# dusk-network/schnorr

Hardware: NVIDIA B200
Metric: verifies_per_s (higher is better)
Workload: dtype u32

## Files before the change

schnorr_b200/csrc/fq.cuh:

```cuda
#pragma once
#include <cstdint>

#include "constants_gen.cuh"

#if defined(__CUDACC__)
#define SB_HD __host__ __device__ __forceinline__
#define SB_D __device__ __forceinline__
#else
#define SB_HD inline
#define SB_D inline
#endif

namespace sb200 {

#ifndef SB_Q1_SHORTCUT
#define SB_Q1_SHORTCUT 0
#endif

struct fq {
  uint32_t v[8];
};

#if !defined(__CUDA_ARCH__)
namespace emu {
struct counters { unsigned long long wide, fq_mul, fq_sqr, fq_addsub, fr_mul, fq_dot5, dfma, fd_mul, fd_sqr, fd_dot5; };
inline counters& cnt() { static thread_local counters c = {}; return c; }
#define SB_COUNT(field, k) (::sb200::emu::cnt().field += (k))
static inline uint32_t add_at(uint32_t* acc, int n, int at, uint64_t val, uint32_t cin) {
  unsigned __int128 carry = cin;
  for (int i = at; i < n; i++) {
    unsigned __int128 t = (unsigned __int128)acc[i] + carry;
    if (i == at) t += (uint32_t)val;
    if (i == at + 1) t += (uint32_t)(val >> 32);
    acc[i] = (uint32_t)t;
    carry = t >> 32;
  }
  return (uint32_t)carry;
}
}
#else
#define SB_COUNT(field, k) ((void)0)
#endif

SB_HD void blk_fold_mac_odd(uint32_t& x0, uint32_t xf, uint32_t tprev, uint32_t* y, uint32_t a, uint32_t b1, uint32_t b3,
                            uint32_t b5, uint32_t b7) {
#if defined(__CUDA_ARCH__)
  asm("{\n\t.reg .u32 t;\n\t"
      "add.cc.u32 t, %10, 0xffffffff;\n\t"
      "addc.cc.u32 %0, %0, %9;\n\t"
      "madc.lo.cc.u32 %1, %11, %12, %1;\n\t"
      "madc.hi.cc.u32 %2, %11, %12, %2;\n\t"
      "madc.lo.cc.u32 %3, %11, %13, %3;\n\t"
      "madc.hi.cc.u32 %4, %11, %13, %4;\n\t"
      "madc.lo.cc.u32 %5, %11, %14, %5;\n\t"
      "madc.hi.cc.u32 %6, %11, %14, %6;\n\t"
      "madc.lo.cc.u32 %7, %11, %15, %7;\n\t"
      "madc.hi.u32 %8, %11, %15, %8;\n\t}"
      : "+r"(x0), "+r"(y[0]), "+r"(y[1]), "+r"(y[2]), "+r"(y[3]), "+r"(y[4]), "+r"(y[5]), "+r"(y[6]), "+r"(y[7])
      : "r"(xf), "r"(tprev), "r"(a), "r"(b1), "r"(b3), "r"(b5), "r"(b7));
#else
  SB_COUNT(wide, 4);
  uint64_t t = (uint64_t)x0 + xf + (tprev != 0 ? 1u : 0u);
  x0 = (uint32_t)t;
  uint32_t c = (uint32_t)(t >> 32);
  c = emu::add_at(y, 8, 0, (uint64_t)a * b1, c);
  c += emu::add_at(y, 8, 2, (uint64_t)a * b3, 0);
  c += emu::add_at(y, 8, 4, (uint64_t)a * b5, 0);
  c += emu::add_at(y, 8, 6, (uint64_t)a * b7, 0);
  (void)c;
#endif
}

SB_HD void blk_mac_even(uint32_t* x, uint32_t& ytop, uint32_t a, uint32_t b0, uint32_t b2, uint32_t b4, uint32_t b6) {
#if defined(__CUDA_ARCH__)
  asm("mad.lo.cc.u32 %0, %9, %10, %0;\n\t"
      "madc.hi.cc.u32 %1, %9, %10, %1;\n\t"
      "madc.lo.cc.u32 %2, %9, %11, %2;\n\t"
      "madc.hi.cc.u32 %3, %9, %11, %3;\n\t"
      "madc.lo.cc.u32 %4, %9, %12, %4;\n\t"
      "madc.hi.cc.u32 %5, %9, %12, %5;\n\t"
      "madc.lo.cc.u32 %6, %9, %13, %6;\n\t"
      "madc.hi.cc.u32 %7, %9, %13, %7;\n\t"
      "addc.u32 %8, %8, 0;"
      : "+r"(x[0]), "+r"(x[1]), "+r"(x[2]), "+r"(x[3]), "+r"(x[4]), "+r"(x[5]), "+r"(x[6]), "+r"(x[7]), "+r"(ytop)
      : "r"(a), "r"(b0), "r"(b2), "r"(b4), "r"(b6));
#else
  SB_COUNT(wide, 4);
  uint32_t c = emu::add_at(x, 8, 0, (uint64_t)a * b0, 0);
  c += emu::add_at(x, 8, 2, (uint64_t)a * b2, 0);
  c += emu::add_at(x, 8, 4, (uint64_t)a * b4, 0);
  c += emu::add_at(x, 8, 6, (uint64_t)a * b6, 0);
  ytop += c;
#endif
}

SB_HD void blk_mac_odd(uint32_t* y, uint32_t a, uint32_t b1, uint32_t b3, uint32_t b5, uint32_t b7) {
#if defined(__CUDA_ARCH__)
  asm("mad.lo.cc.u32 %0, %8, %9, %0;\n\t"
      "madc.hi.cc.u32 %1, %8, %9, %1;\n\t"
      "madc.lo.cc.u32 %2, %8, %10, %2;\n\t"
      "madc.hi.cc.u32 %3, %8, %10, %3;\n\t"
      "madc.lo.cc.u32 %4, %8, %11, %4;\n\t"
      "madc.hi.cc.u32 %5, %8, %11, %5;\n\t"
      "madc.lo.cc.u32 %6, %8, %12, %6;\n\t"
      "madc.hi.u32 %7, %8, %12, %7;"
      : "+r"(y[0]), "+r"(y[1]), "+r"(y[2]), "+r"(y[3]), "+r"(y[4]), "+r"(y[5]), "+r"(y[6]), "+r"(y[7])
      : "r"(a), "r"(b1), "r"(b3), "r"(b5), "r"(b7));
#else
  SB_COUNT(wide, 4);
  uint32_t c = emu::add_at(y, 8, 0, (uint64_t)a * b1, 0);
  c += emu::add_at(y, 8, 2, (uint64_t)a * b3, 0);
  c += emu::add_at(y, 8, 4, (uint64_t)a * b5, 0);
  c += emu::add_at(y, 8, 6, (uint64_t)a * b7, 0);
  (void)c;
#endif
}

SB_HD void blk_red_even_q(uint32_t* x, uint32_t& ytop, uint32_t m, uint32_t q2, uint32_t q4, uint32_t q6) {
#if defined(__CUDA_ARCH__)
  asm("mad.lo.cc.u32 %0, %7, %8, %0;\n\t"
      "madc.hi.cc.u32 %1, %7, %8, %1;\n\t"
      "madc.lo.cc.u32 %2, %7, %9, %2;\n\t"
      "madc.hi.cc.u32 %3, %7, %9, %3;\n\t"
      "madc.lo.cc.u32 %4, %7, %10, %4;\n\t"
      "madc.hi.cc.u32 %5, %7, %10, %5;\n\t"
      "addc.u32 %6, %6, 0;"
      : "+r"(x[2]), "+r"(x[3]), "+r"(x[4]), "+r"(x[5]), "+r"(x[6]), "+r"(x[7]), "+r"(ytop)
      : "r"(m), "r"(q2), "r"(q4), "r"(q6));
#else
  SB_COUNT(wide, 3);
  uint32_t c = emu::add_at(x, 8, 2, (uint64_t)m * q2, 0);
  c += emu::add_at(x, 8, 4, (uint64_t)m * q4, 0);
  c += emu::add_at(x, 8, 6, (uint64_t)m * q6, 0);
  ytop += c;
#endif
}

SB_HD void blk_red_odd_q(uint32_t* y, uint32_t m, uint32_t t0, uint32_t q3, uint32_t q5, uint32_t q7) {
#if defined(__CUDA_ARCH__)
  asm("{\n\t.reg .u32 h;\n\t"
      "min.u32 h, %8, 1;\n\t"
      "sub.u32 h, %8, h;\n\t"
      "add.cc.u32 %0, %0, %9;\n\t"
      "addc.cc.u32 %1, %1, h;\n\t"
      "madc.lo.cc.u32 %2, %8, %10, %2;\n\t"
      "madc.hi.cc.u32 %3, %8, %10, %3;\n\t"
      "madc.lo.cc.u32 %4, %8, %11, %4;\n\t"
      "madc.hi.cc.u32 %5, %8, %11, %5;\n\t"
      "madc.lo.cc.u32 %6, %8, %12, %6;\n\t"
      "madc.hi.u32 %7, %8, %12, %7;\n\t}"
      : "+r"(y[0]), "+r"(y[1]), "+r"(y[2]), "+r"(y[3]), "+r"(y[4]), "+r"(y[5]), "+r"(y[6]), "+r"(y[7])
      : "r"(m), "r"(t0), "r"(q3), "r"(q5), "r"(q7));
#else
  SB_COUNT(wide, 3);
  uint32_t hi1 = m - (m != 0 ? 1u : 0u);
  uint32_t c = emu::add_at(y, 8, 0, ((uint64_t)hi1 << 32) | t0, 0);
  c += emu::add_at(y, 8, 2, (uint64_t)m * q3, 0);
  c += emu::add_at(y, 8, 4, (uint64_t)m * q5, 0);
  c += emu::add_at(y, 8, 6, (uint64_t)m * q7, 0);
  (void)c;
#endif
}

SB_HD void blk_mac1c(uint32_t* acc, uint32_t a, uint32_t b0) {
#if defined(__CUDA_ARCH__)
  asm("mad.lo.cc.u32 %0, %3, %4, %0;\n\t"
      "madc.hi.cc.u32 %1, %3, %4, %1;\n\t"
      "addc.u32 %2, %2, 0;"
      : "+r"(acc[0]), "+r"(acc[1]), "+r"(acc[2])
      : "r"(a), "r"(b0));
#else
  SB_COUNT(wide, 1);
  acc[2] += emu::add_at(acc, 2, 0, (uint64_t)a * b0, 0);
#endif
}
SB_HD void blk_mac2c(uint32_t* acc, uint32_t a, uint32_t b0, uint32_t b1) {
#if defined(__CUDA_ARCH__)
  asm("mad.lo.cc.u32 %0, %5, %6, %0;\n\t"
      "madc.hi.cc.u32 %1, %5, %6, %1;\n\t"
      "madc.lo.cc.u32 %2, %5, %7, %2;\n\t"
      "madc.hi.cc.u32 %3, %5, %7, %3;\n\t"
      "addc.u32 %4, %4, 0;"
      : "+r"(acc[0]), "+r"(acc[1]), "+r"(acc[2]), "+r"(acc[3]), "+r"(acc[4])
      : "r"(a), "r"(b0), "r"(b1));
#else
  SB_COUNT(wide, 2);
  uint32_t c = emu::add_at(acc, 4, 0, (uint64_t)a * b0, 0);
  c += emu::add_at(acc, 4, 2, (uint64_t)a * b1, 0);
  acc[4] += c;
#endif
}
SB_HD void blk_mac3c(uint32_t* acc, uint32_t a, uint32_t b0, uint32_t b1, uint32_t b2) {
#if defined(__CUDA_ARCH__)
  asm("mad.lo.cc.u32 %0, %7, %8, %0;\n\t"
      "madc.hi.cc.u32 %1, %7, %8, %1;\n\t"
      "madc.lo.cc.u32 %2, %7, %9, %2;\n\t"
      "madc.hi.cc.u32 %3, %7, %9, %3;\n\t"
      "madc.lo.cc.u32 %4, %7, %10, %4;\n\t"
      "madc.hi.cc.u32 %5, %7, %10, %5;\n\t"
      "addc.u32 %6, %6, 0;"
      : "+r"(acc[0]), "+r"(acc[1]), "+r"(acc[2]), "+r"(acc[3]), "+r"(acc[4]), "+r"(acc[5]), "+r"(acc[6])
      : "r"(a), "r"(b0), "r"(b1), "r"(b2));
#else
  SB_COUNT(wide, 3);
  uint32_t c = emu::add_at(acc, 6, 0, (uint64_t)a * b0, 0);
  c += emu::add_at(acc, 6, 2, (uint64_t)a * b1, 0);
  c += emu::add_at(acc, 6, 4, (uint64_t)a * b2, 0);
  acc[6] += c;
#endif
}
SB_HD void blk_mac4c(uint32_t* acc, uint32_t a, uint32_t b0, uint32_t b1, uint32_t b2, uint32_t b3) {
  blk_mac_even(acc, acc[8], a, b0, b1, b2, b3);
}

SB_HD void blk_sqr_diag(uint32_t* t, const uint32_t* a) {
#if defined(__CUDA_ARCH__)
  asm("mad.lo.cc.u32 %0, %16, %16, %0;\n\t"
      "madc.hi.cc.u32 %1, %16, %16, %1;\n\t"
      "madc.lo.cc.u32 %2, %17, %17, %2;\n\t"
      "madc.hi.cc.u32 %3, %17, %17, %3;\n\t"
      "madc.lo.cc.u32 %4, %18, %18, %4;\n\t"
      "madc.hi.cc.u32 %5, %18, %18, %5;\n\t"
      "madc.lo.cc.u32 %6, %19, %19, %6;\n\t"
      "madc.hi.cc.u32 %7, %19, %19, %7;\n\t"
      "madc.lo.cc.u32 %8, %20, %20, %8;\n\t"
      "madc.hi.cc.u32 %9, %20, %20, %9;\n\t"
      "madc.lo.cc.u32 %10, %21, %21, %10;\n\t"
      "madc.hi.cc.u32 %11, %21, %21, %11;\n\t"
      "madc.lo.cc.u32 %12, %22, %22, %12;\n\t"
      "madc.hi.cc.u32 %13, %22, %22, %13;\n\t"
      "madc.lo.cc.u32 %14, %23, %23, %14;\n\t"
      "madc.hi.u32 %15, %23, %23, %15;"
      : "+r"(t[0]), "+r"(t[1]), "+r"(t[2]), "+r"(t[3]), "+r"(t[4]), "+r"(t[5]), "+r"(t[6]), "+r"(t[7]), "+r"(t[8]),
        "+r"(t[9]), "+r"(t[10]), "+r"(t[11]), "+r"(t[12]), "+r"(t[13]), "+r"(t[14]), "+r"(t[15])
      : "r"(a[0]), "r"(a[1]), "r"(a[2]), "r"(a[3]), "r"(a[4]), "r"(a[5]), "r"(a[6]), "r"(a[7]));
#else
  SB_COUNT(wide, 8);
  uint32_t c = 0;
  for (int i = 0; i < 8; i++) c += emu::add_at(t, 16, 2 * i, (uint64_t)a[i] * a[i], 0);
  (void)c;
#endif
}

SB_HD void merge_eo16(uint32_t* r, const uint32_t* e, const uint32_t* o) {
#if defined(__CUDA_ARCH__)
  r[0] = e[0];
  asm("add.cc.u32 %0, %15, %30;\n\t"
      "addc.cc.u32 %1, %16, %31;\n\t"
      "addc.cc.u32 %2, %17, %32;\n\t"
      "addc.cc.u32 %3, %18, %33;\n\t"
      "addc.cc.u32 %4, %19, %34;\n\t"
      "addc.cc.u32 %5, %20, %35;\n\t"
      "addc.cc.u32 %6, %21, %36;\n\t"
      "addc.cc.u32 %7, %22, %37;\n\t"
      "addc.cc.u32 %8, %23, %38;\n\t"
      "addc.cc.u32 %9, %24, %39;\n\t"
      "addc.cc.u32 %10, %25, %40;\n\t"
      "addc.cc.u32 %11, %26, %41;\n\t"
      "addc.cc.u32 %12, %27, %42;\n\t"
      "addc.cc.u32 %13, %28, %43;\n\t"
      "addc.u32 %14, %29, %44;"
      : "=r"(r[1]), "=r"(r[2]), "=r"(r[3]), "=r"(r[4]), "=r"(r[5]), "=r"(r[6]), "=r"(r[7]), "=r"(r[8]), "=r"(r[9]),
        "=r"(r[10]), "=r"(r[11]), "=r"(r[12]), "=r"(r[13]), "=r"(r[14]), "=r"(r[15])
      : "r"(e[1]), "r"(e[2]), "r"(e[3]), "r"(e[4]), "r"(e[5]), "r"(e[6]), "r"(e[7]), "r"(e[8]), "r"(e[9]), "r"(e[10]),
        "r"(e[11]), "r"(e[12]), "r"(e[13]), "r"(e[14]), "r"(e[15]), "r"(o[0]), "r"(o[1]), "r"(o[2]), "r"(o[3]), "r"(o[4]),
        "r"(o[5]), "r"(o[6]), "r"(o[7]), "r"(o[8]), "r"(o[9]), "r"(o[10]), "r"(o[11]), "r"(o[12]), "r"(o[13]), "r"(o[14]));
#else
  r[0] = e[0];
  uint64_t c = 0;
  for (int i = 1; i < 16; i++) {
    c += (uint64_t)e[i] + o[i - 1];
    r[i] = (uint32_t)c;
    c >>= 32;
  }
#endif
}

SB_HD uint32_t blk_fold_red_odd(uint32_t& x0, uint32_t xf, uint32_t tprev, uint32_t* y, uint32_t q1, uint32_t q3,
                                uint32_t q5, uint32_t q7) {
  uint32_t m;
#if defined(__CUDA_ARCH__)
  asm("{\n\t.reg .u32 t, h;\n\t"
      "add.cc.u32 t, %11, 0xffffffff;\n\t"
      "addc.cc.u32 %0, %0, %10;\n\t"
      "xor.b32 %9, %0, %12;\n\t"
      "add.u32 %9, %9, 1;\n\t"
      "min.u32 h, %9, 1;\n\t"
      "sub.u32 h, %9, h;\n\t"
      "addc.cc.u32 %1, %1, %0;\n\t"
      "addc.cc.u32 %2, %2, h;\n\t"
      "madc.lo.cc.u32 %3, %9, %13, %3;\n\t"
      "madc.hi.cc.u32 %4, %9, %13, %4;\n\t"
      "madc.lo.cc.u32 %5, %9, %14, %5;\n\t"
      "madc.hi.cc.u32 %6, %9, %14, %6;\n\t"
      "madc.lo.cc.u32 %7, %9, %15, %7;\n\t"
      "madc.hi.u32 %8, %9, %15, %8;\n\t}"
      : "+r"(x0), "+r"(y[0]), "+r"(y[1]), "+r"(y[2]), "+r"(y[3]), "+r"(y[4]), "+r"(y[5]), "+r"(y[6]), "+r"(y[7]), "=&r"(m)
      : "r"(xf), "r"(tprev), "r"(q1), "r"(q3), "r"(q5), "r"(q7));
#else
  SB_COUNT(wide, 4);
  uint64_t t = (uint64_t)x0 + xf + (tprev != 0 ? 1u : 0u);
  x0 = (uint32_t)t;
  uint32_t c = (uint32_t)(t >> 32);
  m = 0u - x0;
  SB_COUNT(wide, -1);
  (void)q1;
  c = emu::add_at(y, 8, 0, ((uint64_t)(m - (m != 0 ? 1u : 0u)) << 32) | x0, c);
  c += emu::add_at(y, 8, 2, (uint64_t)m * q3, 0);
  c += emu::add_at(y, 8, 4, (uint64_t)m * q5, 0);
  c += emu::add_at(y, 8, 6, (uint64_t)m * q7, 0);
  (void)c;
#endif
  return m;
}

SB_HD uint32_t add8(uint32_t* r, const uint32_t* a, const uint32_t* b) {
  uint32_t c;
#if defined(__CUDA_ARCH__)
  asm("add.cc.u32 %0, %9, %17;\n\t"
      "addc.cc.u32 %1, %10, %18;\n\t"
      "addc.cc.u32 %2, %11, %19;\n\t"
      "addc.cc.u32 %3, %12, %20;\n\t"
      "addc.cc.u32 %4, %13, %21;\n\t"
      "addc.cc.u32 %5, %14, %22;\n\t"
      "addc.cc.u32 %6, %15, %23;\n\t"
      "addc.cc.u32 %7, %16, %24;\n\t"
      "addc.u32 %8, 0, 0;"
      : "=r"(r[0]), "=r"(r[1]), "=r"(r[2]), "=r"(r[3]), "=r"(r[4]), "=r"(r[5]), "=r"(r[6]), "=r"(r[7]), "=r"(c)
      : "r"(a[0]), "r"(a[1]), "r"(a[2]), "r"(a[3]), "r"(a[4]), "r"(a[5]), "r"(a[6]), "r"(a[7]), "r"(b[0]), "r"(b[1]),
        "r"(b[2]), "r"(b[3]), "r"(b[4]), "r"(b[5]), "r"(b[6]), "r"(b[7]));
#else
  uint64_t t = 0;
  for (int i = 0; i < 8; i++) {
    t += (uint64_t)a[i] + b[i];
    r[i] = (uint32_t)t;
    t >>= 32;
  }
  c = (uint32_t)t;
#endif
  return c;
}

SB_HD void add8c(uint32_t* r, const uint32_t* a, const uint32_t* b, uint32_t t) {
#if defined(__CUDA_ARCH__)
  asm("{\n\t.reg .u32 t;\n\t"
      "add.cc.u32 t, %24, 0xffffffff;\n\t"
      "addc.cc.u32 %0, %8, %16;\n\t"
      "addc.cc.u32 %1, %9, %17;\n\t"
      "addc.cc.u32 %2, %10, %18;\n\t"
      "addc.cc.u32 %3, %11, %19;\n\t"
      "addc.cc.u32 %4, %12, %20;\n\t"
      "addc.cc.u32 %5, %13, %21;\n\t"
      "addc.cc.u32 %6, %14, %22;\n\t"
      "addc.u32 %7, %15, %23;\n\t}"
      : "=r"(r[0]), "=r"(r[1]), "=r"(r[2]), "=r"(r[3]), "=r"(r[4]), "=r"(r[5]), "=r"(r[6]), "=r"(r[7])
      : "r"(a[0]), "r"(a[1]), "r"(a[2]), "r"(a[3]), "r"(a[4]), "r"(a[5]), "r"(a[6]), "r"(a[7]), "r"(b[0]), "r"(b[1]),
        "r"(b[2]), "r"(b[3]), "r"(b[4]), "r"(b[5]), "r"(b[6]), "r"(b[7]), "r"(t));
#else
  uint64_t c = t != 0 ? 1 : 0;
  for (int i = 0; i < 8; i++) {
    c += (uint64_t)a[i] + b[i];
    r[i] = (uint32_t)c;
    c >>= 32;
  }
#endif
}

SB_HD uint32_t sub8(uint32_t* r, const uint32_t* a, const uint32_t* b) {
  uint32_t c;
#if defined(__CUDA_ARCH__)
  asm("sub.cc.u32 %0, %9, %17;\n\t"
      "subc.cc.u32 %1, %10, %18;\n\t"
      "subc.cc.u32 %2, %11, %19;\n\t"
      "subc.cc.u32 %3, %12, %20;\n\t"
      "subc.cc.u32 %4, %13, %21;\n\t"
      "subc.cc.u32 %5, %14, %22;\n\t"
      "subc.cc.u32 %6, %15, %23;\n\t"
      "subc.cc.u32 %7, %16, %24;\n\t"
      "subc.u32 %8, 0, 0;"
      : "=r"(r[0]), "=r"(r[1]), "=r"(r[2]), "=r"(r[3]), "=r"(r[4]), "=r"(r[5]), "=r"(r[6]), "=r"(r[7]), "=r"(c)
      : "r"(a[0]), "r"(a[1]), "r"(a[2]), "r"(a[3]), "r"(a[4]), "r"(a[5]), "r"(a[6]), "r"(a[7]), "r"(b[0]), "r"(b[1]),
        "r"(b[2]), "r"(b[3]), "r"(b[4]), "r"(b[5]), "r"(b[6]), "r"(b[7]));
#else
  int64_t t = 0;
  for (int i = 0; i < 8; i++) {
    t += (int64_t)a[i] - (int64_t)b[i];
    r[i] = (uint32_t)t;
    t >>= 32;
  }
  c = (uint32_t)t;
#endif
  return c;
}

struct FqP {
  static SB_HD constexpr uint32_t p(int i) {
    constexpr uint32_t t[8] = SB200_FQ_MOD_INIT;
    return t[i];
  }
};
struct FrP {
  static SB_HD constexpr uint32_t p(int i) {
    constexpr uint32_t t[8] = SB200_FR_MOD_INIT;
    return t[i];
  }
  static constexpr uint32_t ninv = SB200_FR_NINV;
};

#if defined(__CUDACC__)
#define SB_X32(v) v, v, v, v, v, v, v, v, v, v, v, v, v, v, v, v, v, v, v, v, v, v, v, v, v, v, v, v, v, v, v, v
__device__ uint32_t d_fq_mod_lane[8 * 32] = {SB_X32(0x00000001u), SB_X32(0xffffffffu), SB_X32(0xfffe5bfeu), SB_X32(0x53bda402u),
                                            SB_X32(0x09a1d805u), SB_X32(0x3339d808u), SB_X32(0x299d7d48u), SB_X32(0x73eda753u)};
__device__ uint32_t d_fr_mod_lane[8 * 32] = {SB_X32(0xd6f72cb7u), SB_X32(0xd0970e5eu), SB_X32(0xccc81082u), SB_X32(0xa6682093u),
                                            SB_X32(0x01343b00u), SB_X32(0x06673b01u), SB_X32(0x6533afa9u), SB_X32(0x0e7db4eau)};
#endif
#ifndef SB_FQ_MOD_IMM
#define SB_FQ_MOD_IMM 1
#endif
#if defined(__CUDACC__)
__constant__ uint32_t c_fq_q1 = 0xffffffffu;
#endif
#if defined(__CUDA_ARCH__) && SB_FQ_MOD_IMM
#define SB_FQ_MOD(i) ((i) == 1 ? c_fq_q1 : FqP::p(i))
#define SB_FR_MOD(i) __ldg(&d_fr_mod_lane[(i) * 32 + (threadIdx.x & 31)])
#elif defined(__CUDA_ARCH__)
#define SB_FQ_MOD(i) __ldg(&d_fq_mod_lane[(i) * 32 + (threadIdx.x & 31)])
#define SB_FR_MOD(i) __ldg(&d_fr_mod_lane[(i) * 32 + (threadIdx.x & 31)])
#else
#define SB_FQ_MOD(i) FqP::p(i)
#define SB_FR_MOD(i) FrP::p(i)
#endif

template <class P>
SB_HD void cond_sub_p(uint32_t* r) {
  uint32_t t[8];
  const uint32_t pp[8] = {P::p(0), P::p(1), P::p(2), P::p(3), P::p(4), P::p(5), P::p(6), P::p(7)};
  uint32_t borrow = sub8(t, r, pp);
#pragma unroll
  for (int i = 0; i < 8; i++) r[i] = borrow ? r[i] : t[i];
}

SB_HD fq fq_zero() {
  fq r;
#pragma unroll
  for (int i = 0; i < 8; i++) r.v[i] = 0;
  return r;
}
SB_HD fq fq_one() {
  const uint32_t c[8] = SB200_FQ_ONE_INIT;
  fq r;
#pragma unroll
  for (int i = 0; i < 8; i++) r.v[i] = c[i];
  return r;
}

SB_HD fq fq_add(const fq& a, const fq& b) {
  SB_COUNT(fq_addsub, 1);
  fq r;
  add8(r.v, a.v, b.v);
  cond_sub_p<FqP>(r.v);
  return r;
}

#ifndef SB_SUB_PREDICATED
#define SB_SUB_PREDICATED 1
#endif
SB_HD fq fq_sub(const fq& a, const fq& b) {
  SB_COUNT(fq_addsub, 1);
  fq r;
  uint32_t borrow = sub8(r.v, a.v, b.v);
#if defined(__CUDA_ARCH__) && SB_SUB_PREDICATED
  asm("{\n\t.reg .pred p;\n\t"
      "setp.ne.u32 p, %8, 0;\n\t"
      "@p add.cc.u32 %0, %0, %9;\n\t"
      "@p addc.cc.u32 %1, %1, %10;\n\t"
      "@p addc.cc.u32 %2, %2, %11;\n\t"
      "@p addc.cc.u32 %3, %3, %12;\n\t"
      "@p addc.cc.u32 %4, %4, %13;\n\t"
      "@p addc.cc.u32 %5, %5, %14;\n\t"
      "@p addc.cc.u32 %6, %6, %15;\n\t"
      "@p addc.u32 %7, %7, %16;\n\t}"
      : "+r"(r.v[0]), "+r"(r.v[1]), "+r"(r.v[2]), "+r"(r.v[3]), "+r"(r.v[4]), "+r"(r.v[5]), "+r"(r.v[6]), "+r"(r.v[7])
      : "r"(borrow), "n"(FqP::p(0)), "n"(FqP::p(1)), "n"(FqP::p(2)), "n"(FqP::p(3)), "n"(FqP::p(4)), "n"(FqP::p(5)), "n"(FqP::p(6)),
        "n"(FqP::p(7)));
  return r;
#endif
  uint32_t t[8];
#pragma unroll
  for (int i = 0; i < 8; i++) t[i] = FqP::p(i) & borrow;
  add8(r.v, r.v, t);
  return r;
}

SB_HD fq fq_neg(const fq& a) { return fq_sub(fq_zero(), a); }

SB_HD fq fq_dbl(const fq& a) { return fq_add(a, a); }

SB_HD bool fq_is_zero(const fq& a) {
  uint32_t o = 0;
#pragma unroll
  for (int i = 0; i < 8; i++) o |= a.v[i];
  return o == 0;
}

SB_HD bool fq_eq(const fq& a, const fq& b) {
  uint32_t o = 0;
#pragma unroll
  for (int i = 0; i < 8; i++) o |= a.v[i] ^ b.v[i];
  return o == 0;
}

SB_HD fq fq_select(const fq& a, const fq& b, bool take_b) {
  fq r;
#pragma unroll
  for (int i = 0; i < 8; i++) r.v[i] = take_b ? b.v[i] : a.v[i];
  return r;
}

SB_HD void mul_wide16(uint32_t* T, const uint32_t* a, const uint32_t* b);
SB_HD fq mont_reduce16(const uint32_t* t);
#ifndef SB_MUL_SEPARATED
#define SB_MUL_SEPARATED 0
#endif
SB_HD fq fq_mul_inl(const fq& a, const fq& b) {
  SB_COUNT(fq_mul, 1);
#if SB_MUL_SEPARATED
  uint32_t T[16];
  mul_wide16(T, a.v, b.v);
  return mont_reduce16(T);
#endif
  uint32_t X[8], Y[8], xf = 0, tprev = 0;
#pragma unroll
  for (int i = 0; i < 8; i++) X[i] = Y[i] = 0;
  const uint32_t q1 = SB_FQ_MOD(1), q2 = SB_FQ_MOD(2), q3 = SB_FQ_MOD(3), q4 = SB_FQ_MOD(4), q5 = SB_FQ_MOD(5),
                 q6 = SB_FQ_MOD(6), q7 = SB_FQ_MOD(7);
#pragma unroll
  for (int i = 0; i < 8; i++) {
    uint32_t ai = a.v[i];
    blk_fold_mac_odd(X[0], xf, tprev, Y, ai, b.v[1], b.v[3], b.v[5], b.v[7]);
    blk_mac_even(X, Y[7], ai, b.v[0], b.v[2], b.v[4], b.v[6]);
    tprev = X[0];
#if defined(__CUDA_ARCH__) && SB_FQ_MOD_IMM
    uint32_t m;
    asm("xor.b32 %0, %1, %2;\n\tadd.u32 %0, %0, 1;" : "=r"(m) : "r"(tprev), "r"(q1));
#else
    uint32_t m = (tprev ^ q1) + 1u;
#endif
    blk_red_even_q(X, Y[7], m, q2, q4, q6);
#if SB_Q1_SHORTCUT
    blk_red_odd_q(Y, m, tprev, q3, q5, q7);
#else
    blk_mac_odd(Y, m, q1, q3, q5, q7);
#endif
    xf = X[1];
    uint32_t nx[8], ny[8];
#pragma unroll
    for (int k = 0; k < 8; k++) nx[k] = Y[k];
#pragma unroll
    for (int k = 0; k < 6; k++) ny[k] = X[k + 2];
    ny[6] = 0;
    ny[7] = 0;
#pragma unroll
    for (int k = 0; k < 8; k++) {
      X[k] = nx[k];
      Y[k] = ny[k];
    }
  }
  fq r;
  uint32_t s[8] = {xf, Y[0], Y[1], Y[2], Y[3], Y[4], Y[5], Y[6]};
  add8c(r.v, X, s, tprev);
  cond_sub_p<FqP>(r.v);
  return r;
}

SB_HD fq mont_reduce16(const uint32_t* t) {
  uint32_t X[8], Y[8], xf = 0, tprev = 0;
#pragma unroll
  for (int i = 0; i < 8; i++) {
    X[i] = t[i];
    Y[i] = 0;
  }
  const uint32_t q1 = SB_FQ_MOD(1), q2 = SB_FQ_MOD(2), q3 = SB_FQ_MOD(3), q4 = SB_FQ_MOD(4), q5 = SB_FQ_MOD(5),
                 q6 = SB_FQ_MOD(6), q7 = SB_FQ_MOD(7);
#pragma unroll
  for (int i = 0; i < 8; i++) {
    uint32_t m = blk_fold_red_odd(X[0], xf, tprev, Y, q1, q3, q5, q7);
    tprev = X[0];
    blk_red_even_q(X, Y[7], m, q2, q4, q6);
    xf = X[1];
    uint32_t nx[8], ny[8];
#pragma unroll
    for (int k = 0; k < 8; k++) nx[k] = Y[k];
#pragma unroll
    for (int k = 0; k < 6; k++) ny[k] = X[k + 2];
    ny[6] = 0;
    ny[7] = 0;
#pragma unroll
    for (int k = 0; k < 8; k++) {
      X[k] = nx[k];
      Y[k] = ny[k];
    }
  }
  fq v, r;
  uint32_t s[8] = {xf, Y[0], Y[1], Y[2], Y[3], Y[4], Y[5], Y[6]};
  add8c(v.v, X, s, tprev);
  add8(r.v, v.v, t + 8);
  cond_sub_p<FqP>(r.v);
  return r;
}

SB_HD fq fq_sqr_inl(const fq& x) {
  SB_COUNT(fq_sqr, 1);
  const uint32_t* a = x.v;
  uint32_t E[16], O[16];
#pragma unroll
  for (int i = 0; i < 16; i++) E[i] = O[i] = 0;
  blk_mac4c(O + 0, a[0], a[1], a[3], a[5], a[7]);
  blk_mac3c(E + 2, a[0], a[2], a[4], a[6]);
  blk_mac3c(O + 2, a[1], a[2], a[4], a[6]);
  blk_mac3c(E + 4, a[1], a[3], a[5], a[7]);
  blk_mac3c(O + 4, a[2], a[3], a[5], a[7]);
  blk_mac2c(E + 6, a[2], a[4], a[6]);
  blk_mac2c(O + 6, a[3], a[4], a[6]);
  blk_mac2c(E + 8, a[3], a[5], a[7]);
  blk_mac2c(O + 8, a[4], a[5], a[7]);
  blk_mac1c(E + 10, a[4], a[6]);
  blk_mac1c(O + 10, a[5], a[6]);
  blk_mac1c(E + 12, a[5], a[7]);
  blk_mac1c(O + 12, a[6], a[7]);
  uint32_t S[16], T[16];
  merge_eo16(S, E, O);
  T[0] = S[0] << 1;
#pragma unroll
  for (int i = 1; i < 16; i++) T[i] = (S[i] << 1) | (S[i - 1] >> 31);
  blk_sqr_diag(T, a);
  return mont_reduce16(T);
}

SB_HD void mul_wide16(uint32_t* T, const uint32_t* a, const uint32_t* b) {
  uint32_t E[18], O[18];
#pragma unroll
  for (int i = 0; i < 18; i++) E[i] = O[i] = 0;
#pragma unroll
  for (int i = 0; i < 8; i++) {
    if ((i & 1) == 0) {
      blk_mac4c(E + i, a[i], b[0], b[2], b[4], b[6]);
      blk_mac4c(O + i, a[i], b[1], b[3], b[5], b[7]);
    } else {
      blk_mac4c(O + i - 1, a[i], b[0], b[2], b[4], b[6]);
      blk_mac4c(E + i + 1, a[i], b[1], b[3], b[5], b[7]);
    }
  }
  merge_eo16(T, E, O);
}

SB_HD void acc17(uint32_t* S, const uint32_t* T) {
#if defined(__CUDA_ARCH__)
  asm("add.cc.u32 %0, %0, %17;\n\t"
      "addc.cc.u32 %1, %1, %18;\n\t"
      "addc.cc.u32 %2, %2, %19;\n\t"
      "addc.cc.u32 %3, %3, %20;\n\t"
      "addc.cc.u32 %4, %4, %21;\n\t"
      "addc.cc.u32 %5, %5, %22;\n\t"
      "addc.cc.u32 %6, %6, %23;\n\t"
      "addc.cc.u32 %7, %7, %24;\n\t"
      "addc.cc.u32 %8, %8, %25;\n\t"
      "addc.cc.u32 %9, %9, %26;\n\t"
      "addc.cc.u32 %10, %10, %27;\n\t"
      "addc.cc.u32 %11, %11, %28;\n\t"
      "addc.cc.u32 %12, %12, %29;\n\t"
      "addc.cc.u32 %13, %13, %30;\n\t"
      "addc.cc.u32 %14, %14, %31;\n\t"
      "addc.cc.u32 %15, %15, %32;\n\t"
      "addc.u32 %16, %16, 0;"
      : "+r"(S[0]), "+r"(S[1]), "+r"(S[2]), "+r"(S[3]), "+r"(S[4]), "+r"(S[5]), "+r"(S[6]), "+r"(S[7]), "+r"(S[8]),
        "+r"(S[9]), "+r"(S[10]), "+r"(S[11]), "+r"(S[12]), "+r"(S[13]), "+r"(S[14]), "+r"(S[15]), "+r"(S[16])
      : "r"(T[0]), "r"(T[1]), "r"(T[2]), "r"(T[3]), "r"(T[4]), "r"(T[5]), "r"(T[6]), "r"(T[7]), "r"(T[8]), "r"(T[9]),
        "r"(T[10]), "r"(T[11]), "r"(T[12]), "r"(T[13]), "r"(T[14]), "r"(T[15]));
#else
  uint64_t c = 0;
  for (int i = 0; i < 16; i++) {
    c += (uint64_t)S[i] + T[i];
    S[i] = (uint32_t)c;
    c >>= 32;
  }
  S[16] += (uint32_t)c;
#endif
}

SB_HD fq mont_reduce17(const uint32_t* S) {
  uint32_t X[8], Y[8], xf = 0, tprev = 0;
#pragma unroll
  for (int i = 0; i < 8; i++) {
    X[i] = S[i];
    Y[i] = 0;
  }
  const uint32_t q1 = SB_FQ_MOD(1), q2 = SB_FQ_MOD(2), q3 = SB_FQ_MOD(3), q4 = SB_FQ_MOD(4), q5 = SB_FQ_MOD(5),
                 q6 = SB_FQ_MOD(6), q7 = SB_FQ_MOD(7);
#pragma unroll
  for (int i = 0; i < 8; i++) {
    uint32_t m = blk_fold_red_odd(X[0], xf, tprev, Y, q1, q3, q5, q7);
    tprev = X[0];
    blk_red_even_q(X, Y[7], m, q2, q4, q6);
    xf = X[1];
    uint32_t nx[8], ny[8];
#pragma unroll
    for (int k = 0; k < 8; k++) nx[k] = Y[k];
#pragma unroll
    for (int k = 0; k < 6; k++) ny[k] = X[k + 2];
    ny[6] = 0;
    ny[7] = 0;
#pragma unroll
    for (int k = 0; k < 8; k++) {
      X[k] = nx[k];
      Y[k] = ny[k];
    }
  }
  fq v, r;
  uint32_t s[8] = {xf, Y[0], Y[1], Y[2], Y[3], Y[4], Y[5], Y[6]};
  add8c(v.v, X, s, tprev);
  uint32_t top = S[16] + add8(r.v, v.v, S + 8);
  uint32_t t[8], q2x[8];
#pragma unroll
  for (int i = 0; i < 8; i++) q2x[i] = (FqP::p(i) << 1) | (i ? FqP::p(i - 1) >> 31 : 0u);
  uint32_t borrow = sub8(t, r.v, q2x);
  bool ge = (top != 0) | (borrow == 0);
#pragma unroll
  for (int i = 0; i < 8; i++) r.v[i] = ge ? t[i] : r.v[i];
  cond_sub_p<FqP>(r.v);
  return r;
}

SB_HD void merge_eo17(uint32_t* S, const uint32_t* E, const uint32_t* O) {
  S[0] = E[0];
#if defined(__CUDA_ARCH__)
  asm("add.cc.u32 %0, %16, %32;\n\t"
      "addc.cc.u32 %1, %17, %33;\n\t"
      "addc.cc.u32 %2, %18, %34;\n\t"
      "addc.cc.u32 %3, %19, %35;\n\t"
      "addc.cc.u32 %4, %20, %36;\n\t"
      "addc.cc.u32 %5, %21, %37;\n\t"
      "addc.cc.u32 %6, %22, %38;\n\t"
      "addc.cc.u32 %7, %23, %39;\n\t"
      "addc.cc.u32 %8, %24, %40;\n\t"
      "addc.cc.u32 %9, %25, %41;\n\t"
      "addc.cc.u32 %10, %26, %42;\n\t"
      "addc.cc.u32 %11, %27, %43;\n\t"
      "addc.cc.u32 %12, %28, %44;\n\t"
      "addc.cc.u32 %13, %29, %45;\n\t"
      "addc.cc.u32 %14, %30, %46;\n\t"
      "addc.u32 %15, %31, %47;"
      : "=r"(S[1]), "=r"(S[2]), "=r"(S[3]), "=r"(S[4]), "=r"(S[5]), "=r"(S[6]), "=r"(S[7]), "=r"(S[8]), "=r"(S[9]), "=r"(S[10]),
        "=r"(S[11]), "=r"(S[12]), "=r"(S[13]), "=r"(S[14]), "=r"(S[15]), "=r"(S[16])
      : "r"(E[1]), "r"(E[2]), "r"(E[3]), "r"(E[4]), "r"(E[5]), "r"(E[6]), "r"(E[7]), "r"(E[8]), "r"(E[9]), "r"(E[10]), "r"(E[11]),
        "r"(E[12]), "r"(E[13]), "r"(E[14]), "r"(E[15]), "r"(E[16]), "r"(O[0]), "r"(O[1]), "r"(O[2]), "r"(O[3]), "r"(O[4]), "r"(O[5]),
        "r"(O[6]), "r"(O[7]), "r"(O[8]), "r"(O[9]), "r"(O[10]), "r"(O[11]), "r"(O[12]), "r"(O[13]), "r"(O[14]), "r"(O[15]));
#else
  uint64_t c = 0;
  for (int i = 1; i < 17; i++) {
    c += (uint64_t)E[i] + O[i - 1];
    S[i] = (uint32_t)c;
    c >>= 32;
  }
#endif
}

#ifndef SB_DOT5_ROWMAJOR
#define SB_DOT5_ROWMAJOR 1
#endif
SB_HD fq fq_dot5_inl(const uint32_t (*cst)[8], const fq& s0, const fq& s1, const fq& s2, const fq& s3, const fq& s4) {
  SB_COUNT(fq_dot5, 1);
#if SB_DOT5_ROWMAJOR
  {
    uint32_t E[18], O[18], S[17];
#pragma unroll
    for (int i = 0; i < 18; i++) E[i] = O[i] = 0;
    const fq* sv[5] = {&s0, &s1, &s2, &s3, &s4};
#pragma unroll
    for (int i = 0; i < 8; i++) {
#pragma unroll
      for (int j = 0; j < 5; j++) {
        const uint32_t a = sv[j]->v[i];
        if ((i & 1) == 0) {
          blk_mac4c(E + i, a, cst[j][0], cst[j][2], cst[j][4], cst[j][6]);
          blk_mac4c(O + i, a, cst[j][1], cst[j][3], cst[j][5], cst[j][7]);
        } else {
          blk_mac4c(O + i - 1, a, cst[j][0], cst[j][2], cst[j][4], cst[j][6]);
          blk_mac4c(E + i + 1, a, cst[j][1], cst[j][3], cst[j][5], cst[j][7]);
        }
      }
    }
    merge_eo17(S, E, O);
    return mont_reduce17(S);
  }
#endif
  uint32_t S[17], T[16], c[8];
#pragma unroll
  for (int i = 0; i < 17; i++) S[i] = 0;
  const fq* sv[5] = {&s0, &s1, &s2, &s3, &s4};
#pragma unroll
  for (int j = 0; j < 5; j++) {
#pragma unroll
    for (int i = 0; i < 8; i++) c[i] = cst[j][i];
    mul_wide16(T, sv[j]->v, c);
    acc17(S, T);
  }
  return mont_reduce17(S);
}

#ifndef SB_MUL_NOINLINE
#define SB_MUL_NOINLINE 1
#endif
#if defined(__CUDACC__) && SB_MUL_NOINLINE
#ifndef SB_MUL_BYPTR
#define SB_MUL_BYPTR 0
#endif
#if SB_MUL_BYPTR
static __device__ __noinline__ void fq_mul_ptr(fq* r, const fq* a, const fq* b) { *r = fq_mul_inl(*a, *b); }
static __device__ __noinline__ void fq_sqr_ptr(fq* r, const fq* a) { *r = fq_sqr_inl(*a); }
static __device__ __forceinline__ fq fq_mul_ool(const fq& a, const fq& b) { fq r; fq_mul_ptr(&r, &a, &b); return r; }
static __device__ __forceinline__ fq fq_sqr_ool(const fq& a) { fq r; fq_sqr_ptr(&r, &a); return r; }
#else
static __device__ __noinline__ fq fq_mul_ool(fq a, fq b) { return fq_mul_inl(a, b); }
static __device__ __noinline__ fq fq_sqr_ool(fq a) { return fq_sqr_inl(a); }
#endif
static __device__ __noinline__ fq fq_dot5_ool(const uint32_t (*cst)[8], fq s0, fq s1, fq s2, fq s3, fq s4) {
  return fq_dot5_inl(cst, s0, s1, s2, s3, s4);
}
#endif
SB_HD fq fq_mul(const fq& a, const fq& b) {
#if defined(__CUDA_ARCH__) && SB_MUL_NOINLINE
  return fq_mul_ool(a, b);
#else
  return fq_mul_inl(a, b);
#endif
}
SB_HD fq fq_dot5(const uint32_t (*cst)[8], const fq& s0, const fq& s1, const fq& s2, const fq& s3, const fq& s4) {
#if defined(__CUDA_ARCH__) && SB_MUL_NOINLINE
  return fq_dot5_ool(cst, s0, s1, s2, s3, s4);
#else
  return fq_dot5_inl(cst, s0, s1, s2, s3, s4);
#endif
}
SB_HD fq fq_sqr(const fq& a) {
#if defined(__CUDA_ARCH__) && SB_MUL_NOINLINE
  return fq_sqr_ool(a);
#else
  return fq_sqr_inl(a);
#endif
}

#ifndef SB_PAIRED_MUL
#define SB_PAIRED_MUL 0
#endif
struct fq2 {
  fq a, b;
};
#if defined(__CUDACC__) && SB_MUL_NOINLINE
static __device__ __noinline__ fq2 fq_mul2_ool(fq a, fq b, fq c, fq d) {
  fq2 r;
  r.a = fq_mul_inl(a, b);
  r.b = fq_mul_inl(c, d);
  return r;
}
static __device__ __noinline__ fq2 fq_sqr2_ool(fq a, fq b) {
  fq2 r;
  r.a = fq_sqr_inl(a);
  r.b = fq_sqr_inl(b);
  return r;
}
#endif
SB_HD void fq_mul2(const fq& a, const fq& b, const fq& c, const fq& d, fq& r0, fq& r1) {
#if defined(__CUDA_ARCH__) && SB_MUL_NOINLINE && SB_PAIRED_MUL
  fq2 r = fq_mul2_ool(a, b, c, d);
  r0 = r.a;
  r1 = r.b;
#else
  r0 = fq_mul(a, b);
  r1 = fq_mul(c, d);
#endif
}
SB_HD void fq_sqr2(const fq& a, const fq& b, fq& r0, fq& r1) {
#if defined(__CUDA_ARCH__) && SB_MUL_NOINLINE && SB_PAIRED_MUL
  fq2 r = fq_sqr2_ool(a, b);
  r0 = r.a;
  r1 = r.b;
#else
  r0 = fq_sqr(a);
  r1 = fq_sqr(b);
#endif
}

SB_HD fq fq_to_mont(const fq& a) {
  const fq r2 = {SB200_FQ_R2_INIT};
  return fq_mul(a, r2);
}
SB_HD fq fq_from_mont(const fq& a) {
  fq one = fq_zero();
  one.v[0] = 1;
  return fq_mul(a, one);
}

SB_HD fq fq_inv(const fq& a) {
  fq tab[16];
  tab[0] = fq_one();
  tab[1] = a;
#pragma unroll 1
  for (int i = 2; i < 16; i++) tab[i] = fq_mul(tab[i - 1], a);
  const uint32_t e[8] = {0xffffffffu, 0xfffffffeu, 0xfffe5bfeu, 0x53bda402u, 0x09a1d805u, 0x3339d808u, 0x299d7d48u, 0x73eda753u};
  fq acc = fq_one();
#pragma unroll 1
  for (int w = 63; w >= 0; w--) {
    acc = fq_sqr(acc);
    acc = fq_sqr(acc);
    acc = fq_sqr(acc);
    acc = fq_sqr(acc);
    uint32_t d = (e[w >> 3] >> ((w & 7) * 4)) & 15u;
    acc = fq_mul(acc, tab[d]);
  }
  return acc;
}

struct fr {
  uint32_t v[8];
};

SB_HD fr fr_mont_mul(const fr& a, const fr& b) {
  SB_COUNT(fr_mul, 1);
  uint32_t X[8], Y[8], xf = 0;
#pragma unroll
  for (int i = 0; i < 8; i++) X[i] = Y[i] = 0;
#pragma unroll
  for (int i = 0; i < 8; i++) {
    uint32_t ai = a.v[i];
    blk_fold_mac_odd(X[0], xf, 0u, Y, ai, b.v[1], b.v[3], b.v[5], b.v[7]);
    blk_mac_even(X, Y[7], ai, b.v[0], b.v[2], b.v[4], b.v[6]);
    uint32_t m = X[0] * FrP::ninv;
    blk_mac_even(X, Y[7], m, SB_FR_MOD(0), SB_FR_MOD(2), SB_FR_MOD(4), SB_FR_MOD(6));
    blk_mac_odd(Y, m, SB_FR_MOD(1), SB_FR_MOD(3), SB_FR_MOD(5), SB_FR_MOD(7));
    xf = X[1];
    uint32_t nx[8], ny[8];
#pragma unroll
    for (int k = 0; k < 8; k++) nx[k] = Y[k];
#pragma unroll
    for (int k = 0; k < 6; k++) ny[k] = X[k + 2];
    ny[6] = 0;
    ny[7] = 0;
#pragma unroll
    for (int k = 0; k < 8; k++) {
      X[k] = nx[k];
      Y[k] = ny[k];
    }
  }
  fr r;
  uint32_t s[8] = {xf, Y[0], Y[1], Y[2], Y[3], Y[4], Y[5], Y[6]};
  add8(r.v, X, s);
  cond_sub_p<FrP>(r.v);
  return r;
}

SB_HD fr fr_mul(const fr& a, const fr& b) {
  const fr r2 = {SB200_FR_R2_INIT};
  return fr_mont_mul(fr_mont_mul(a, b), r2);
}

SB_HD fr fr_sub(const fr& a, const fr& b) {
  fr r;
  uint32_t borrow = sub8(r.v, a.v, b.v);
  uint32_t t[8];
#pragma unroll
  for (int i = 0; i < 8; i++) t[i] = FrP::p(i) & borrow;
  add8(r.v, r.v, t);
  return r;
}

}
```

Baseline: 28.84 million.

## Interleave Montgomery reduction into field squaring with pre-doubled operands

Replaces the separate compute-product, double, add-diagonal, then reduce16 squaring with a row-by-row squaring that interleaves Montgomery reduction steps, using pre-doubled limbs so the doubling pass disappears. The first row folds a0*a0 directly into the reduction seed. It also trims one instruction from the odd fold-reduction step. The goal is fewer instructions and registers in the hot fq squaring. In exchange it adds a pre-reduction of inputs with the top bit set, so doubled limbs fit, and more complex carry bookkeeping.

```diff
diff --git a/schnorr_b200/csrc/fq.cuh b/schnorr_b200/csrc/fq.cuh
--- a/schnorr_b200/csrc/fq.cuh
+++ b/schnorr_b200/csrc/fq.cuh
@@ -211,35 +211,6 @@
 }
 SB_HD void blk_mac4c(uint32_t* acc, uint32_t a, uint32_t b0, uint32_t b1, uint32_t b2, uint32_t b3) {
   blk_mac_even(acc, acc[8], a, b0, b1, b2, b3);
-}
-
-SB_HD void blk_sqr_diag(uint32_t* t, const uint32_t* a) {
-#if defined(__CUDA_ARCH__)
-  asm("mad.lo.cc.u32 %0, %16, %16, %0;\n\t"
-      "madc.hi.cc.u32 %1, %16, %16, %1;\n\t"
-      "madc.lo.cc.u32 %2, %17, %17, %2;\n\t"
-      "madc.hi.cc.u32 %3, %17, %17, %3;\n\t"
-      "madc.lo.cc.u32 %4, %18, %18, %4;\n\t"
-      "madc.hi.cc.u32 %5, %18, %18, %5;\n\t"
-      "madc.lo.cc.u32 %6, %19, %19, %6;\n\t"
-      "madc.hi.cc.u32 %7, %19, %19, %7;\n\t"
-      "madc.lo.cc.u32 %8, %20, %20, %8;\n\t"
-      "madc.hi.cc.u32 %9, %20, %20, %9;\n\t"
-      "madc.lo.cc.u32 %10, %21, %21, %10;\n\t"
-      "madc.hi.cc.u32 %11, %21, %21, %11;\n\t"
-      "madc.lo.cc.u32 %12, %22, %22, %12;\n\t"
-      "madc.hi.cc.u32 %13, %22, %22, %13;\n\t"
-      "madc.lo.cc.u32 %14, %23, %23, %14;\n\t"
-      "madc.hi.u32 %15, %23, %23, %15;"
-      : "+r"(t[0]), "+r"(t[1]), "+r"(t[2]), "+r"(t[3]), "+r"(t[4]), "+r"(t[5]), "+r"(t[6]), "+r"(t[7]), "+r"(t[8]),
-        "+r"(t[9]), "+r"(t[10]), "+r"(t[11]), "+r"(t[12]), "+r"(t[13]), "+r"(t[14]), "+r"(t[15])
-      : "r"(a[0]), "r"(a[1]), "r"(a[2]), "r"(a[3]), "r"(a[4]), "r"(a[5]), "r"(a[6]), "r"(a[7]));
-#else
-  SB_COUNT(wide, 8);
-  uint32_t c = 0;
-  for (int i = 0; i < 8; i++) c += emu::add_at(t, 16, 2 * i, (uint64_t)a[i] * a[i], 0);
-  (void)c;
-#endif
 }
 
 SB_HD void merge_eo16(uint32_t* r, const uint32_t* e, const uint32_t* o) {
@@ -283,10 +254,9 @@
   asm("{\n\t.reg .u32 t, h;\n\t"
       "add.cc.u32 t, %11, 0xffffffff;\n\t"
       "addc.cc.u32 %0, %0, %10;\n\t"
-      "xor.b32 %9, %0, %12;\n\t"
-      "add.u32 %9, %9, 1;\n\t"
-      "min.u32 h, %9, 1;\n\t"
-      "sub.u32 h, %9, h;\n\t"
+      "xor.b32 h, %0, %12;\n\t"
+      "add.u32 %9, h, 1;\n\t"
+      "min.u32 h, h, %9;\n\t"
       "addc.cc.u32 %1, %1, %0;\n\t"
       "addc.cc.u32 %2, %2, h;\n\t"
       "madc.lo.cc.u32 %3, %9, %13, %3;\n\t"
@@ -609,32 +579,153 @@
   return r;
 }
 
+template <int N>
+SB_HD void blk_mac_top(uint32_t* x, uint32_t& ytop, uint32_t a, const uint32_t* b) {
+  uint32_t t[2 * N + 1];
+#pragma unroll
+  for (int k = 0; k < 2 * N; k++) t[k] = x[8 - 2 * N + k];
+  t[2 * N] = ytop;
+  if constexpr (N == 1) blk_mac1c(t, a, b[0]);
+  if constexpr (N == 2) blk_mac2c(t, a, b[0], b[1]);
+  if constexpr (N == 3) blk_mac3c(t, a, b[0], b[1], b[2]);
+  if constexpr (N == 4) blk_mac4c(t, a, b[0], b[1], b[2], b[3]);
+#pragma unroll
+  for (int k = 0; k < 2 * N; k++) x[8 - 2 * N + k] = t[k];
+  ytop = t[2 * N];
+}
+
+SB_HD void blk_sqr_top(uint32_t* y, uint32_t a6, uint32_t a7) {
+#if defined(__CUDA_ARCH__)
+  asm("mad.lo.cc.u32 %0, %4, %4, %0;\n\t"
+      "madc.hi.cc.u32 %1, %4, %4, %1;\n\t"
+      "madc.lo.cc.u32 %2, %5, %5, %2;\n\t"
+      "madc.hi.u32 %3, %5, %5, %3;"
+      : "+r"(y[4]), "+r"(y[5]), "+r"(y[6]), "+r"(y[7])
+      : "r"(a6), "r"(a7));
+#else
+  SB_COUNT(wide, 2);
+  uint32_t c = emu::add_at(y, 8, 4, (uint64_t)a6 * a6, 0);
+  c += emu::add_at(y, 8, 6, (uint64_t)a7 * a7, 0);
+  (void)c;
+#endif
+}
+
+SB_HD void sqr_red_shift(uint32_t* X, uint32_t* Y, uint32_t& xf, uint32_t& tprev, uint32_t q1, uint32_t q2, uint32_t q3,
+                         uint32_t q4, uint32_t q5, uint32_t q6, uint32_t q7) {
+  uint32_t m = blk_fold_red_odd(X[0], xf, tprev, Y, q1, q3, q5, q7);
+  tprev = X[0];
+  blk_red_even_q(X, Y[7], m, q2, q4, q6);
+  xf = X[1];
+  uint32_t nx[8], ny[8];
+#pragma unroll
+  for (int k = 0; k < 8; k++) nx[k] = Y[k];
+#pragma unroll
+  for (int k = 0; k < 6; k++) ny[k] = X[k + 2];
+  ny[6] = 0;
+  ny[7] = 0;
+#pragma unroll
+  for (int k = 0; k < 8; k++) {
+    X[k] = nx[k];
+    Y[k] = ny[k];
+  }
+}
+
+SB_HD void blk_sqr_row0(uint32_t* X, uint32_t* Y, uint32_t& xf, uint32_t& tprev, uint32_t a0, uint32_t q1, uint32_t q2,
+                        uint32_t q3, uint32_t q4, uint32_t q5, uint32_t q6, uint32_t q7) {
+#if defined(__CUDA_ARCH__)
+  const uint64_t s = (uint64_t)a0 * a0;
+  tprev = (uint32_t)s;
+  xf = (uint32_t)(s >> 32);
+  uint32_t m, h;
+  asm("xor.b32 %1, %2, %3;\n\tadd.u32 %0, %1, 1;\n\tmin.u32 %1, %1, %0;" : "=&r"(m), "=&r"(h) : "r"(tprev), "r"(q1));
+  const uint64_t p[6] = {(uint64_t)m * q3, (uint64_t)m * q5, (uint64_t)m * q7, (uint64_t)m * q2, (uint64_t)m * q4, (uint64_t)m * q6};
+  X[0] = tprev;
+  X[1] = h;
+#pragma unroll
+  for (int k = 0; k < 3; k++) {
+    X[2 + 2 * k] = (uint32_t)p[k];
+    X[3 + 2 * k] = (uint32_t)(p[k] >> 32);
+    Y[2 * k] = (uint32_t)p[3 + k];
+    Y[2 * k + 1] = (uint32_t)(p[3 + k] >> 32);
+  }
+  Y[6] = Y[7] = 0;
+#else
+  SB_COUNT(wide, 7);
+  (void)q1;
+  const uint64_t s = (uint64_t)a0 * a0;
+  tprev = (uint32_t)s;
+  xf = (uint32_t)(s >> 32);
+  const uint32_t m = 0u - tprev;
+  const uint64_t p[6] = {(uint64_t)m * q3, (uint64_t)m * q5, (uint64_t)m * q7, (uint64_t)m * q2, (uint64_t)m * q4, (uint64_t)m * q6};
+  X[0] = tprev;
+  X[1] = m - (m != 0 ? 1u : 0u);
+  for (int k = 0; k < 3; k++) {
+    X[2 + 2 * k] = (uint32_t)p[k];
+    X[3 + 2 * k] = (uint32_t)(p[k] >> 32);
+    Y[2 * k] = (uint32_t)p[3 + k];
+    Y[2 * k + 1] = (uint32_t)(p[3 + k] >> 32);
+  }
+  Y[6] = Y[7] = 0;
+#endif
+}
+
 SB_HD fq fq_sqr_inl(const fq& x) {
   SB_COUNT(fq_sqr, 1);
-  const uint32_t* a = x.v;
-  uint32_t E[16], O[16];
-#pragma unroll
-  for (int i = 0; i < 16; i++) E[i] = O[i] = 0;
-  blk_mac4c(O + 0, a[0], a[1], a[3], a[5], a[7]);
-  blk_mac3c(E + 2, a[0], a[2], a[4], a[6]);
-  blk_mac3c(O + 2, a[1], a[2], a[4], a[6]);
-  blk_mac3c(E + 4, a[1], a[3], a[5], a[7]);
-  blk_mac3c(O + 4, a[2], a[3], a[5], a[7]);
-  blk_mac2c(E + 6, a[2], a[4], a[6]);
-  blk_mac2c(O + 6, a[3], a[4], a[6]);
-  blk_mac2c(E + 8, a[3], a[5], a[7]);
-  blk_mac2c(O + 8, a[4], a[5], a[7]);
-  blk_mac1c(E + 10, a[4], a[6]);
-  blk_mac1c(O + 10, a[5], a[6]);
-  blk_mac1c(E + 12, a[5], a[7]);
-  blk_mac1c(O + 12, a[6], a[7]);
-  uint32_t S[16], T[16];
-  merge_eo16(S, E, O);
-  T[0] = S[0] << 1;
-#pragma unroll
-  for (int i = 1; i < 16; i++) T[i] = (S[i] << 1) | (S[i - 1] >> 31);
-  blk_sqr_diag(T, a);
-  return mont_reduce16(T);
+  fq s = x;
+  if (s.v[7] >> 31) {
+    const uint32_t qq[8] = {FqP::p(0), FqP::p(1), FqP::p(2), FqP::p(3), FqP::p(4), FqP::p(5), FqP::p(6), FqP::p(7)};
+    sub8(s.v, s.v, qq);
+    if (s.v[7] >> 31) sub8(s.v, s.v, qq);
+  }
+  const uint32_t* a = s.v;
+  uint32_t as[8], d[8];
+#pragma unroll
+  for (int j = 1; j < 8; j++) {
+    as[j] = a[j] << 1;
+    d[j] = as[j] | (a[j - 1] >> 31);
+  }
+  const uint32_t q1 = SB_FQ_MOD(1), q2 = SB_FQ_MOD(2), q3 = SB_FQ_MOD(3), q4 = SB_FQ_MOD(4), q5 = SB_FQ_MOD(5),
+                 q6 = SB_FQ_MOD(6), q7 = SB_FQ_MOD(7);
+  uint32_t X[8], Y[8], xf, tprev;
+  blk_sqr_row0(X, Y, xf, tprev, a[0], q1, q2, q3, q4, q5, q6, q7);
+  {
+    const uint32_t bx[4] = {as[1], d[3], d[5], d[7]};
+    blk_mac_top<4>(X, Y[7], a[0], bx);
+    blk_mac3c(Y, a[0], d[2], d[4], d[6]);
+  }
+#pragma unroll
+  for (int i = 1; i < 7; i++) {
+    sqr_red_shift(X, Y, xf, tprev, q1, q2, q3, q4, q5, q6, q7);
+    uint32_t b[8];
+    b[i - 1] = a[i];
+    b[i] = as[i + 1];
+#pragma unroll
+    for (int j = i + 2; j < 8; j++) b[j - 1] = d[j];
+    const int rx = (i - 1) & 1 ? i : i - 1, ry = (i - 1) & 1 ? i - 1 : i;
+    const uint32_t bx[4] = {b[rx], b[rx + 2 < 7 ? rx + 2 : 6], b[rx + 4 < 7 ? rx + 4 : 6], b[6]};
+    const uint32_t by[3] = {b[ry], b[ry + 2 < 6 ? ry + 2 : 5], b[5]};
+    if (i == 6) {
+      blk_mac_top<1>(X, Y[7], a[6], bx);
+      blk_sqr_top(Y, a[6], a[7]);
+      continue;
+    }
+    switch ((8 - rx) / 2) {
+      case 4: blk_mac_top<4>(X, Y[7], a[i], bx); break;
+      case 3: blk_mac_top<3>(X, Y[7], a[i], bx); break;
+      default: blk_mac_top<2>(X, Y[7], a[i], bx); break;
+    }
+    switch ((7 - ry) / 2) {
+      case 3: blk_mac3c(Y, a[i], by[0], by[1], by[2]); break;
+      case 2: blk_mac2c(Y + 2, a[i], by[0], by[1]); break;
+      default: blk_mac1c(Y + 4, a[i], by[0]); break;
+    }
+  }
+  sqr_red_shift(X, Y, xf, tprev, q1, q2, q3, q4, q5, q6, q7);
+  fq r;
+  uint32_t t[8] = {xf, Y[0], Y[1], Y[2], Y[3], Y[4], Y[5], Y[6]};
+  add8c(r.v, X, t, tprev);
+  cond_sub_p<FqP>(r.v);
+  return r;
 }
 
 SB_HD void mul_wide16(uint32_t* T, const uint32_t* a, const uint32_t* b) {
```

Measured after the change: 29.37 million, median of 6. 1.9% higher.
